# noc-lab/sac-expert

Measured on AMD Instinct MI355X. Metric: SAC gradient-steps/sec (batch=256, 256x2 MLP), higher is better.
Workload: dtype f32; 1 GPU; HalfCheetah-v3-shaped synthetic buffer, SAC twin-Q + actor + alpha update (no model), fp32; obs_dim=17, act_dim=6, batch=256, buffer_rows=1000000, parallelism=replicas x1 (independent seeds, no collective), seeds_per_gpu=1, sampler=NumPy-legacy MT19937 stream on device (bit-exact indices)

## Files before the change

sac-expert_amd/csrc/k_sac.hip:

```cpp
#include <hip/hip_runtime.h>
#include <cstddef>
#include <cstdio>
#include <cstdlib>
#include <type_traits>
#include <utility>
#include <math.h>
#include "sacx_internal.h"

#pragma clang fp contract(off)

namespace sacx {

typedef float floatx4 __attribute__((ext_vector_type(4)));


typedef __bf16 bf16x8_t __attribute__((ext_vector_type(8)));
__device__ __forceinline__ floatx4 mfma_bf16_2slab(const float (&a0)[4], const float (&a1)[4], const float (&b0)[4],
                                                   const float (&b1)[4], floatx4 c) {
    const bf16x8_t av = {(__bf16)a0[0], (__bf16)a0[1], (__bf16)a0[2], (__bf16)a0[3],
                         (__bf16)a1[0], (__bf16)a1[1], (__bf16)a1[2], (__bf16)a1[3]};
    const bf16x8_t bv = {(__bf16)b0[0], (__bf16)b0[1], (__bf16)b0[2], (__bf16)b0[3],
                         (__bf16)b1[0], (__bf16)b1[1], (__bf16)b1[2], (__bf16)b1[3]};
    return __builtin_amdgcn_mfma_f32_16x16x32_bf16(av, bv, c, 0, 0, 0);
}
// ... 651 lines not shown
            if (f.nt > 0) ak = 0.5f * ak;
            const float lk = ak / (float)f.mb;
            tot = k == 0 ? lk : tot + lk;
        }
        const int64_t seq = f.ctl->mfit_seq;
        f.mstats[(size_t)(seq % f.mstats_cap) * 2] = tot;
        f.mstats[(size_t)(seq % f.mstats_cap) * 2 + 1] = (float)seq;
        f.ctl->t_model = t_model + 1;
        f.ctl->mfit_seq = seq + 1;
    }
}

template <int MODE, int NQ>
__device__ __forceinline__ void qhead_block(const QHeadArgs& q, int block, int64_t so, const FinalArgs* fin = nullptr);
template <int NQ, int OW = 0, int FIN = 0>
__device__ __forceinline__ void actor_head_body(const HeadArgs& h, const FinalArgs& f, int block, int64_t so,
                                                const FinalArgs& ffin);
template <int NQ, int OW = 0>
__device__ __forceinline__ void actor_head_body(const HeadArgs& h, const FinalArgs& f, int block, int64_t so) {
    actor_head_body<NQ, OW, 0>(h, f, block, so, f);
}

__device__ __forceinline__ int xcd_tile(int b, int T) {
    const int x = b & 7, j = b >> 3, q = T >> 3, r = T & 7;
    return x * q + (x < r ? x : r) + j;
}

struct HeadPre {
    float xs[4], u, ls, am, ad, bias;
    float4 pv[4];
};
__device__ __forceinline__ void head_pre_load(const HeadArgs& hd, const GemmProb& g, int m0, int64_t so, bool parts,
                                              HeadPre& p) {
    const int t = threadIdx.x, row = t >> 4, col = t & 15;
    const int A = hd.A, Aout = hd.Aout, H1 = hd.H1, S = g.K - A;
    HeadSeg sg = hd.seg[0];
    reloc(sg, so);
    const bool rok = m0 + row < g.M;
    const __amdgpu_buffer_rsrc_t rx = make_rsrc(g.A, 0x7fffffffu);
#pragma unroll
    for (int q = 0; q < 4; ++q) p.xs[q] = bload(rx, boff(rok && col + 16 * q < S, (m0 + row) * g.lda + col + 16 * q));
    const bool jok = col < A;
    p.u = bload(rs(sg.noise), boff(jok && rok, (m0 + row - sg.r0) * A + col));
    p.ls = bload(rs(sr(hd.logstd, so)), boff(jok && !hd.per_state_std, col));
    p.am = bload(rs(sr(hd.a_mean, so)), boff(jok, col));
    p.ad = bload(rs(sr(hd.a_den, so)), boff(jok, col));
    const __amdgpu_buffer_rsrc_t rw3 = make_rsrc(sr(hd.W3, so), 0x7fffffffu);
    p.bias = bload(rw3, boff(col < Aout, H1 * Aout + col));
    if (parts) {
        const __amdgpu_buffer_rsrc_t rp = rs(sr(hd.part, so));
        const bool pok = rok && col < Aout;
#pragma unroll
        for (int i = 0; i < 4; ++i) p.pv[i] = bload4(rp, boff(pok && 4 * i < hd.tq, ((m0 + row) * Aout + col) * hd.tq + 4 * i));
    }
}
__device__ __forceinline__ float head_pre_mu(const HeadPre& p) {
    float v = 0.f;
#pragma unroll
    for (int i = 0; i < 4; ++i) {
        v = v + p.pv[i].x; v = v + p.pv[i].y; v = v + p.pv[i].z; v = v + p.pv[i].w;
    }
    return v + p.bias;
}
__device__ __forceinline__ void head_pre_finish(const HeadArgs& hd, const GemmProb& g, int m0, int tn,
                                                float (&As)[16][68], const HeadPre& p, float mu, int64_t so) {
    const int t = threadIdx.x, lane = t & 63;
    const int row = t >> 4, col = t & 15;
    const int A = hd.A, S = g.K - A;
    HeadSeg sg = hd.seg[0];
    reloc(sg, so);
    const bool rok = m0 + row < g.M;
    const bool jok = col < A;
    const float lv = __shfl(mu, (lane & ~15) | min(col + A, 15), 64);
    const float lraw = hd.per_state_std ? lv : p.ls;
    float nv = 0.f, nc = 0.f, pin = 0.f;
    if (jok) {
        const float l = fminf(fmaxf(lraw, -5.f), 2.f);
        const float sd = expf(l);
        const float x = mu + sd * p.u;
        const float th = tanhf(x);
        const float pi = hd.lim * th;
        const float z = (x - mu) / expf(l);
        nv = z * z + 2.f * l + LOG2PI_F;
        nc = 2.f * ((LN2_F - x) - softplus_f(-2.f * x));
        pin = (pi - p.am) / p.ad;
    }
    nv += __shfl_xor(nv, 8, 16);
    nv += __shfl_xor(nv, 4, 16);
    nv += __shfl_xor(nv, 2, 16);
    nv += __shfl_xor(nv, 1, 16);
    nc += __shfl_xor(nc, 8, 16);
    nc += __shfl_xor(nc, 4, 16);
    nc += __shfl_xor(nc, 2, 16);
    nc += __shfl_xor(nc, 1, 16);
    if (tn == 0 && col == 0 && rok && sg.nlp_out != nullptr) sg.nlp_out[m0 + row - sg.r0] = 0.5f * nv + nc;
#pragma unroll
    for (int q = 0; q < 4; ++q)
        if (col + 16 * q < S) As[row][col + 16 * q] = p.xs[q];
    if (jok) As[row][S + col] = pin;
}

template <bool SYNC = true>
__device__ __forceinline__ void head_prologue(const HeadArgs& hd, const GemmProb& g, int m0, int tn,
                                              float (&As)[16][68], float (&red)[4][4][64], int64_t so) {
    const int t = threadIdx.x, wave = t >> 6, lane = t & 63, r = lane & 15, grp = lane >> 4;
    const int row = t >> 4, col = t & 15;
    const int Aout = hd.Aout, H1 = hd.H1;
    HeadPre p;
    head_pre_load(hd, g, m0, so, hd.part != nullptr, p);
    float mu;
    if (hd.part != nullptr) {
        mu = head_pre_mu(p);
    } else {
        const __amdgpu_buffer_rsrc_t rw3 = make_rsrc(sr(hd.W3, so), 0x7fffffffu);
        const __amdgpu_buffer_rsrc_t rh = make_rsrc(sr(hd.H2, so), 0x7fffffffu);
        const int nIt = H1 >> 4, per = (nIt + 3) >> 2, i0 = wave * per, i1 = min(nIt, i0 + per);
        const bool hm = m0 + r < g.M, wn = r < Aout;
        floatx4 c0 = {0.f, 0.f, 0.f, 0.f}, c1 = {0.f, 0.f, 0.f, 0.f};
        for (int it = i0; it < i1; it += 4) {
            float a[4][4], b[4][4];
#pragma unroll
            for (int u4 = 0; u4 < 4; ++u4) {
                const bool ok = it + u4 < i1;
                const int k0 = (it + u4) * 16 + grp * 4;
                const float4 v = bload4(rh, boff(ok && hm, (m0 + r) * hd.ldh + k0));
                a[u4][0] = v.x; a[u4][1] = v.y; a[u4][2] = v.z; a[u4][3] = v.w;
#pragma unroll
                for (int j = 0; j < 4; ++j) b[u4][j] = bload(rw3, boff(ok && wn, (k0 + j) * Aout + r));
            }
            __builtin_amdgcn_sched_barrier(0);
#pragma unroll
            for (int u4 = 0; u4 < 4; ++u4) {
                c0 = __builtin_amdgcn_mfma_f32_16x16x4f32(a[u4][0], b[u4][0], c0, 0, 0, 0);
                c1 = __builtin_amdgcn_mfma_f32_16x16x4f32(a[u4][1], b[u4][1], c1, 0, 0, 0);
                c0 = __builtin_amdgcn_mfma_f32_16x16x4f32(a[u4][2], b[u4][2], c0, 0, 0, 0);
                c1 = __builtin_amdgcn_mfma_f32_16x16x4f32(a[u4][3], b[u4][3], c1, 0, 0, 0);
            }
        }
        const floatx4 acc = c0 + c1;
#pragma unroll
        for (int q = 0; q < 4; ++q) red[wave][q][lane] = acc[q];
        __syncthreads();
        const int L = ((row >> 2) << 4) | col, R = row & 3;
        float v = red[0][R][L] + red[1][R][L];
        v = v + red[2][R][L];
        v = v + red[3][R][L];
        mu = v + p.bias;
    }
    head_pre_finish(hd, g, m0, tn, As, p, mu, so);
    if constexpr (SYNC) __syncthreads();
}

__device__ __forceinline__ void head_bwd_prologue(HeadBwdArgs hb, int m0, int tn, float (&d3s)[16][17], int64_t so) {
    reloc(hb, so);
    const int t = threadIdx.x, lane = t & 63, row = t >> 4, col = t & 15;
    const int B = hb.B, A = hb.A;
    const int m = m0 + row;
    const bool rok = m < B + hb.ne, jok = col < A, ok = rok && jok;
    const bool pol = m < B;
    const int ci = m * A + col;
    const float ct = bload(rs(hb.c_t), boff(ok, ci));
    const float sd = bload(rs(hb.c_std), boff(ok, ci));
    const float u = bload(rs(hb.c_u), boff(ok, ci));
    const float mk = bload(rs(hb.c_mask), boff(ok, ci));
    const float ad = bload(rs(pol ? hb.a_den : hb.ma_den), boff(jok, col));
    const __amdgpu_buffer_rsrc_t rg = rs(hb.gpol);
    const float g0 = bload(rg, boff(rok && pol, m));
    const float g1 = bload(rg, boff(rok && pol, B + m));
    const float alpha = bload(rs(hb.alpha), 0u);
    const float eps = hb.ctl != nullptr ? bload(rs(reinterpret_cast<const float*>(hb.ctl)),
                                               (uint32_t)offsetof(Ctl, epsilon)) : 0.f;
    const __amdgpu_buffer_rsrc_t rp = rs(hb.part), rm = rs(hb.mpart);
    const int tq = hb.tq, tqm = hb.tqm, e = m - B;
    float4 v0[4], v1[4], vm[8];
#pragma unroll
    for (int i = 0; i < 4; ++i) {
        const bool iok = ok && pol && 4 * i < tq;
        v0[i] = bload4(rp, boff(iok, (m * A + col) * tq + 4 * i));
        v1[i] = bload4(rp, boff(iok, ((B + m) * A + col) * tq + 4 * i));
    }
#pragma unroll
    for (int i = 0; i < 8; ++i) vm[i] = bload4(rm, boff(ok && !pol && 4 * i < tqm, (e * A + col) * tqm + 4 * i));
// ... 401 lines not shown
    static_assert(GEMM_MAXP == 8, "one pin per problem's tile_begin");
    const uint32_t kf = khdr_flags(kh);
    if (kf & 0x80u) {
        total_tiles = (int)khdr_field(kh, 0);
        row_blocks = (int)khdr_field(kh, 1);
        tb[0] = 0;
#pragma unroll
        for (int i = 1; i < GEMM_MAXP; ++i) tb[i] = (int)khdr_field(kh, i + 1);
        nprob = (int)(kf & 15u);
        has_final = (int)((kf >> 4) & 3u);
        xcd_map = (int)((kf >> 6) & 1u);
    } else {
        has_final = ga.has_final; row_blocks = ga.row_blocks; total_tiles = ga.total_tiles;
        xcd_map = ga.xcd_map; nprob = ga.nprob;
#pragma unroll
        for (int i = 0; i < GEMM_MAXP; ++i) tb[i] = ga.probs[i].tile_begin;
        asm volatile("" ::"s"(has_final), "s"(row_blocks), "s"(total_tiles), "s"(xcd_map), "s"(nprob),
                     "s"(tb[1]), "s"(tb[2]), "s"(tb[3]), "s"(tb[4]), "s"(tb[5]), "s"(tb[6]), "s"(tb[7]));
    }
    int tile = (int)blockIdx.x - (has_final ? 1 : 0);
    if (tile < 0) {
        FinalArgs f = ga.fin;
        reloc(f, so);
        finalize_update(f, f.nred);
        return;
    }
    if constexpr (gemm_rows_head(MODE, ROWK)) {
        if (tile < row_blocks) {
            actor_head_body<NQ>(ga.head, ga.hfin, ga.head_block0 + tile, so);
            return;
        }
        tile -= row_blocks;
    }
    if (tile >= total_tiles) {
        if constexpr (gemm_rows_qhead(MODE, ROWK)) {
            qhead_block<gemm_qhead_mode(ROWK), NQ>(ga.qh, tile - total_tiles, so, ROWK == GR_QHEAD ? &ga.fin : nullptr);
        } else if constexpr (gemm_rows_mfinal(ROWK)) {
            if (ga.has_mfinal == 2) {
                FinalArgs f = ga.fin;
                reloc(f, so);
                bc_finalize(f);
            } else if (ga.has_mfinal) {
                mfit_final(ga.mfin, &ga.adam, ga.p_stride);
            }
        }
        return;
    }
    if (xcd_map) tile = xcd_tile(tile, total_tiles);
    int p = 0;
#pragma unroll
    for (int i = 1; i < GEMM_MAXP; ++i)
        if (i < nprob && tile >= tb[i]) p = i;
    GemmProb g = ga.probs[p];
    if constexpr (MODE == GM_FWD && ROWK == GR_ACTOR_HEAD) {
        const HeadArgs& hd = ga.head;
        const HeadSeg& s0 = hd.seg[0];
        asm volatile("" ::"s"(g.A), "s"(g.B), "s"(g.lda), "s"(g.ldb), "s"(g.M), "s"(g.N), "s"(g.K), "s"(g.tiles_n),
                     "s"(g.tile_begin), "s"(g.act), "s"(g.bias), "s"(g.headp), "s"(hd.H2), "s"(hd.W3), "s"(hd.logstd),
                     "s"(hd.a_mean), "s"(hd.a_den), "s"(hd.ldh), "s"(hd.H1), "s"(hd.A), "s"(hd.Aout),
                     "s"(hd.per_state_std), "s"(hd.lim), "s"(s0.r0), "s"(s0.noise), "s"(s0.nlp_out), "s"(g.vec),
                     "s"(hd.part), "s"(hd.tq));
    } else if constexpr (MODE == GM_FWD && ROWK == GR_HEAD_PART) {
        asm volatile("" ::"s"(g.A), "s"(g.B), "s"(g.lda), "s"(g.ldb), "s"(g.M), "s"(g.N), "s"(g.K), "s"(g.tiles_n),
                     "s"(g.tile_begin), "s"(g.act), "s"(g.bias), "s"(g.vec), "s"(g.C), "s"(g.ldc),
                     "s"(g.pw), "s"(g.ppart), "s"(g.pw_ld), "s"(g.pw_cs), "s"(g.pw_n));
    } else if constexpr (MODE == GM_FWD) {
        asm volatile("" ::"s"(g.A), "s"(g.B), "s"(g.lda), "s"(g.ldb), "s"(g.M), "s"(g.N), "s"(g.K), "s"(g.tiles_n),
                     "s"(g.tile_begin), "s"(g.act), "s"(g.bias), "s"(g.mse), "s"(g.se_raw), "s"(g.spe_raw),
                     "s"(g.dmean), "s"(g.dden), "s"(g.headp), "s"(g.vec));
    } else if constexpr (MODE == GM_DX && ROWK == GR_PIQHEAD) {
// ... 55 lines not shown
        e2 = g.P[pidx + 2 * ga.p_stride];
        e3 = bload(make_rsrc(g.T, g.T != nullptr ? 0x7fffffffu : 0u), (uint32_t)pidx * 4u);
    }
    EpiScalars es{};
    if constexpr (MODE == GM_DW || (MODE == GM_FWD && ROWK == GR_MSE_HEAD))
        es = epi_scalars(sr(ga.ctl, so), g.group);
    constexpr bool PART = gemm_rows_part(MODE, ROWK);
    float pwv[8];
    if constexpr (PART) {
        const __amdgpu_buffer_rsrc_t rpw = rs(g.pw);
#pragma unroll
        for (int j = 0; j < 8; ++j) pwv[j] = bload(rpw, boff(j < g.pw_n && nn < g.N, j * g.pw_ld + nnc * g.pw_cs));
    }

    const int nIt = (g.K + 15) >> 4;
    const int per = (nIt + 3) >> 2;
    const int it0 = wave * per;
    const int it1 = min(nIt, it0 + per);
    const int m = m0 + r, n = n0 + r;
    const bool mok = m < g.M, nok = n < g.N;

    const __amdgpu_buffer_rsrc_t ra = make_rsrc(g.A, 0x7fffffffu);
    const __amdgpu_buffer_rsrc_t rb = make_rsrc(g.B, 0x7fffffffu);
    const __amdgpu_buffer_rsrc_t rw = rs(g.wgen);
    floatx4 acc0 = {0.f, 0.f, 0.f, 0.f};
    floatx4 acc1 = {0.f, 0.f, 0.f, 0.f};
    __shared__ float As[16][68];
    bool a_lds = false;
    if constexpr (MODE == GM_FWD && ROWK == GR_ACTOR_HEAD) {
        if (g.headp) {
            float bp[4];
            const int k0 = it0 * 16 + grp * 4;
            load_b<BKC, false, false>(rb, g, n, nok, it0 < it1 ? k0 : (1 << 30), bp);
            head_prologue(ga.head, g, m0, tn, As, red, so);
            if (it0 < it1) {
                float a[4];
#pragma unroll
                for (int j = 0; j < 4; ++j) a[j] = (k0 + j < g.K) ? As[r][k0 + j] : 0.f;
                if constexpr (BF) {
                    const float z[4] = {0.f, 0.f, 0.f, 0.f};
                    acc0 = mfma_bf16_2slab(a, z, bp, z, acc0);
                } else {
                    acc0 = __builtin_amdgcn_mfma_f32_16x16x4f32(a[0], bp[0], acc0, 0, 0, 0);
                    acc1 = __builtin_amdgcn_mfma_f32_16x16x4f32(a[1], bp[1], acc1, 0, 0, 0);
                    acc0 = __builtin_amdgcn_mfma_f32_16x16x4f32(a[2], bp[2], acc0, 0, 0, 0);
                    acc1 = __builtin_amdgcn_mfma_f32_16x16x4f32(a[3], bp[3], acc1, 0, 0, 0);
                }
            }
            a_lds = true;
        }
    }
    __shared__ float d3s[ROWK == GR_HEAD_BWD ? 16 : 1][17];
    if constexpr (MODE == GM_DX && ROWK == GR_HEAD_BWD) {
        auto hbw_loop = [&](auto vt) {
            constexpr bool V = decltype(vt)::value;
            const int Aout = ga.hbw.Aout;
            float a[4][4], b[4][4], w[4][2];
#pragma unroll
            for (int u = 0; u < 4; ++u) {
                const int it = it0 + u;
                const int k0 = it * 16 + grp * 4;
                const int k0e = it < it1 ? k0 : (1 << 30);
                load_a<true, V, false>(ra, g, m, mok, k0e, a[u], rw);
                load_b<true, V>(rb, g, n, nok, k0e, b[u]);
                const int kr = it * 16 + r;
#pragma unroll
                for (int s = 0; s < 2; ++s)
// ... 753 lines not shown

template <bool PK, bool T32>
static void launch_gemm_t(const GemmArgs& a, hipStream_t s) {
    const std::make_integer_sequence<int, GR_COUNT> rows;
    switch (a.mode) {
    case GM_FWD: return launch_gemm_rows<GM_FWD, PK, T32>(a, s, rows);
    case GM_DX: return launch_gemm_rows<GM_DX, PK, T32>(a, s, rows);
    case GM_DW: return launch_gemm_rows<GM_DW, PK, T32>(a, s, rows);
    default: gemm_variant_die(a);
    }
}

#ifndef SACX_FWD2_NW
#define SACX_FWD2_NW 16
#endif

#ifndef SACX_DW_DIAG_XBF
#define SACX_DW_DIAG_XBF 0
#endif
#ifndef SACX_FWD2_STAMP
#define SACX_FWD2_STAMP 0
#endif

#define F2_STAMP(P)                                                                          \
    do {                                                                                     \
        if (SACX_FWD2_STAMP == (P) && ga.ktime != nullptr) {                                 \
            __syncthreads();                                                                 \
            if (threadIdx.x == 0) {                                                          \
                ga.ktime[2 * f2_slot(ga, g1, lt, HEAD)] = t0;                                \
                ga.ktime[2 * f2_slot(ga, g1, lt, HEAD) + 1] = __builtin_amdgcn_s_memrealtime(); \
            }                                                                                \
        }                                                                                    \
    } while (0)
__device__ __forceinline__ int f2_slot(const GemmArgs& ga, const GemmProb& g1, int lt, bool head) {
    return (head ? ga.row_blocks : 0) + g1.tile_begin + lt;
}
template <int VEC, int NW, bool HEAD, int FIN = 0, int H0X = 256, bool GATHER = false>
__global__ __launch_bounds__(NW * 64, HEAD ? 2 * NW / 4 : 1) void k_fwd2(GemmArgs ga) {
    constexpr int L0T = (H0X / 16) / NW, CTW = 16 / NW, PU = H0X / 64;
    const uint64_t t0 = __builtin_amdgcn_s_memrealtime();
    __shared__ float hs[16][H0X + 4];
    __shared__ float red2[4][4][4][64];
    int p = (int)blockIdx.y;
    if constexpr (HEAD) {
        if (p == 0) {
            const int tile = (int)blockIdx.x;
            if (tile >= ga.row_blocks) return;
            const int blk = ga.head_block0 + (NW / 4) * tile;
            actor_head_body<4, 0, FIN>(ga.head, ga.hfin, blk, 0, ga.fin);
            if (ga.ktime != nullptr) {
                __syncthreads();
                if (threadIdx.x == 0) {
                    ga.ktime[2 * tile] = t0;
                    ga.ktime[2 * tile + 1] = __builtin_amdgcn_s_memrealtime();
                }
            }
            return;
        }
        --p;
    }
    const GemmProb g0 = ga.probs[2 * p], g1 = ga.probs[2 * p + 1];
    const int lt = (int)blockIdx.x;
    if (lt >= ((g1.M + 15) >> 4) * g1.tiles_n) return;
    if (SACX_FWD2_STAMP == 3) {
        asm volatile("" ::"s"(g0.N), "s"(g1.N), "s"(g0.A), "s"(g1.B));
        F2_STAMP(3);
    }
    const int tm = lt / g1.tiles_n, cg = lt - tm * g1.tiles_n;
    const int m0 = tm * 16;
    const int wave = wave_id(), lane = threadIdx.x & 63, r = lane & 15, grp = lane >> 4;
    const int kq = wave & 3, ch = wave >> 2;
    const bool headp = HEAD && g0.headp;
    const int m = m0 + r;
    const bool mok = m < g0.M;
    const int H0 = g0.N, N1 = g1.N;
    const int nIt0 = (g0.K + 15) >> 4;
    const int per1 = (H0 + 63) >> 6;

    HeadPre hpre;
    if constexpr (HEAD)
        if (headp && threadIdx.x < 256) head_pre_load(ga.head, g0, m0, 0, true, hpre);
    const __amdgpu_buffer_rsrc_t rx = make_rsrc(g0.A, 0x7fffffffu);
    const __amdgpu_buffer_rsrc_t rw0 = make_rsrc(g0.B, 0x7fffffffu);
    const __amdgpu_buffer_rsrc_t rw1 = make_rsrc(g1.B, 0x7fffffffu);
    const __amdgpu_buffer_rsrc_t rnull = rs(nullptr);
    float xa[2][4];
    const float* trec = nullptr;
    if constexpr (GATHER) {
        const MGatherArgs& mg = ga.mg;
        const int64_t seq = mg.ctl->mfit_seq, start = mg.ctl->start;
        const int32_t* ir = mg.idx_ring + (seq % mg.idx_cap) * (int64_t)(mg.nm * mg.mb) + (int64_t)p * mg.mb;
        auto rec_of = [&](int rr) {
            int64_t phys = start + ir[min(rr, g0.M - 1)];
            phys = phys >= mg.cap ? phys - mg.cap : phys;
            return mg.replay + phys * (int64_t)mg.stride;
        };
        const float* grow = rec_of(m);
        trec = rec_of(m0 + ((threadIdx.x & 255) >> 4));
#pragma unroll
        for (int s2 = 0; s2 < 2; ++s2) {
            const int k0 = s2 < nIt0 ? s2 * 16 + grp * 4 : (1 << 30);
            const bool live = mok && k0 < g0.K;
            const int kb = k0 < g0.K ? k0 : 0;
            float raw[4];
            if constexpr (VEC == 1) {
                const float4 q = *reinterpret_cast<const float4*>(grow + kb);
                raw[0] = q.x; raw[1] = q.y; raw[2] = q.z; raw[3] = q.w;
            } else {
#pragma unroll
                for (int j = 0; j < 4; ++j) raw[j] = grow[min(kb + j, g0.K - 1)];
            }
#pragma unroll
            for (int j = 0; j < 4; ++j) {
                const int kc = min(kb + j, g0.K - 1);
                const float* mu = kc < mg.S ? mg.s_mean + kc : mg.a_mean + (kc - mg.S);
                const float* den = kc < mg.S ? mg.s_den + kc : mg.a_den + (kc - mg.S);
                float x = (raw[j] - *mu) / *den;
                asm("" : "+v"(x));
                xa[s2][j] = (live && kb + j < g0.K) ? x : 0.f;
            }
            if (cg == 0 && wave == 0 && mok && k0 < g0.lda)
                *reinterpret_cast<float4*>(const_cast<float*>(g0.A) + (size_t)m * g0.lda + k0) =
                    float4{xa[s2][0], xa[s2][1], xa[s2][2], xa[s2][3]};
        }
    } else {
#pragma unroll
        for (int s2 = 0; s2 < 2; ++s2)
            load_a<true, VEC == 1, false>(rx, g0, m, mok && !headp, s2 < nIt0 ? s2 * 16 + grp * 4 : (1 << 30), xa[s2], rnull);
    }
    float w0[L0T][2][4], b0[L0T];
#pragma unroll
    for (int i = 0; i < L0T; ++i) {
        const int c = wave + NW * i;
        const int nc = 16 * c + r;
        const bool cok = nc < H0;
#pragma unroll
        for (int s2 = 0; s2 < 2; ++s2) load_b<false, false>(rw0, g0, nc, cok, s2 < nIt0 && cok ? s2 * 16 + grp * 4 : (1 << 30), w0[i][s2]);
        b0[i] = bload(rs(g0.bias), boff(cok, nc));
    }
    float w1[CTW][PU][4];
#pragma unroll
    for (int j2 = 0; j2 < CTW; ++j2) {
        const int ct = CTW * ch + j2;
        const int n1 = 64 * cg + 16 * ct + r;
        const bool nok = n1 < N1;
#pragma unroll
        for (int u = 0; u < PU; ++u) {
            const int it = kq * per1 + u;
            load_b<false, false>(rw1, g1, n1, nok, u < per1 ? it * 16 + grp * 4 : (1 << 30), w1[j2][u]);
        }
    }
    const int te = threadIdx.x & 255, eh = threadIdx.x >> 8;
    const int row = te >> 4, col = te & 15;
    float b1[CTW];
    constexpr int NPW = HEAD ? 1 : 8;
    float pwv[CTW][NPW];
#pragma unroll
    for (int j2 = 0; j2 < CTW; ++j2) {
        const int nn = 64 * cg + 16 * (CTW * eh + j2) + col;
        b1[j2] = bload(rs(g1.bias), boff(nn < N1, nn));
        if constexpr (!HEAD) {
            const __amdgpu_buffer_rsrc_t rpw = rs(ga.rowk == GR_HEAD_PART ? g1.pw : nullptr);
#pragma unroll
            for (int j = 0; j < NPW; ++j)
                pwv[j2][j] = bload(rpw, boff(j < g1.pw_n && nn < N1, j * g1.pw_ld + min(nn, N1 - 1) * g1.pw_cs));
        }
    }
    __builtin_amdgcn_sched_barrier(0);
    if constexpr (GATHER) {
        const MGatherArgs& mg = ga.mg;
        const int S = mg.S, A = mg.A, tcol = 16 * eh + col, mmr = m0 + row;
        if (cg == 0 && mmr < g0.M && tcol <= S) {
            const int c = tcol;
            const float traw0 = c < S ? trec[S + A + c] : trec[2 * S + A];
            const float traw1 = c < S ? trec[c] : 0.f;
            const float tmu = c < S ? mg.d_mean[c] : mg.r_norm[0];
            const float tden = c < S ? mg.d_den[c] : mg.r_norm[1];
            float y = c < S ? ((traw0 - traw1) - tmu) / tden : (traw0 - tmu) / tden;
            const float cl = c < S ? mg.clip_d : mg.clip_r;
            if (cl > 0.f) y = fminf(fmaxf(y, -cl), cl);
            mg.T[(size_t)(p * mg.mb + mmr) * (S + 1) + c] = y;
        }
    }
    if constexpr (HEAD) {
        __shared__ float As[16][68];
        if (headp) {
            if (SACX_FWD2_STAMP == 6) {
                const float mu6 = head_pre_mu(hpre);
                asm volatile("" ::"v"(mu6), "v"(hpre.xs[3]), "v"(hpre.u));
                F2_STAMP(6);
            }
            if (threadIdx.x < 256) head_pre_finish(ga.head, g0, m0, cg, As, hpre, head_pre_mu(hpre), 0);
            __syncthreads();
            F2_STAMP(5);
#pragma unroll
            for (int s2 = 0; s2 < 2; ++s2)
#pragma unroll
                for (int j = 0; j < 4; ++j) {
                    const int k = s2 * 16 + grp * 4 + j;
                    xa[s2][j] = (s2 < nIt0 && k < g0.K) ? As[r][k] : 0.f;
                }
        }
    }

#pragma unroll
    for (int i = 0; i < L0T; ++i) {
        const int c = wave + NW * i;
        if (16 * c >= H0) break;
        floatx4 ps[2];
#pragma unroll
        for (int s2 = 0; s2 < 2; ++s2) {
            floatx4 x0 = {0.f, 0.f, 0.f, 0.f}, x1 = {0.f, 0.f, 0.f, 0.f};
            x0 = __builtin_amdgcn_mfma_f32_16x16x4f32(xa[s2][0], w0[i][s2][0], x0, 0, 0, 0);
            x1 = __builtin_amdgcn_mfma_f32_16x16x4f32(xa[s2][1], w0[i][s2][1], x1, 0, 0, 0);
            x0 = __builtin_amdgcn_mfma_f32_16x16x4f32(xa[s2][2], w0[i][s2][2], x0, 0, 0, 0);
            x1 = __builtin_amdgcn_mfma_f32_16x16x4f32(xa[s2][3], w0[i][s2][3], x1, 0, 0, 0);
            ps[s2] = x0 + x1;
        }
        const floatx4 v4 = ((ps[0] + ps[1]) + floatx4{0.f, 0.f, 0.f, 0.f}) + floatx4{0.f, 0.f, 0.f, 0.f};
        const int nc = 16 * c + r;
#pragma unroll
        for (int q = 0; q < 4; ++q) {
            const float h = act_f(v4[q] + b0[i], g0.act);
            hs[4 * grp + q][nc] = h;
            const int mm = m0 + 4 * grp + q;
            if (cg == 0 && mm < g0.M && nc < H0) st_out(&g0.C[(size_t)mm * g0.ldc + nc], h);
        }
    }
    F2_STAMP(1);
    __syncthreads();

    float a1[PU][4];
#pragma unroll
    for (int u = 0; u < PU; ++u) {
        const int k0 = (kq * per1 + u) * 16 + grp * 4;
        const float4 q4 = u < per1 ? *reinterpret_cast<const float4*>(&hs[r][k0]) : float4{0.f, 0.f, 0.f, 0.f};
        a1[u][0] = q4.x; a1[u][1] = q4.y; a1[u][2] = q4.z; a1[u][3] = q4.w;
    }
#pragma unroll
    for (int j2 = 0; j2 < CTW; ++j2) {
        floatx4 acc0 = {0.f, 0.f, 0.f, 0.f}, acc1 = {0.f, 0.f, 0.f, 0.f};
#pragma unroll
        for (int u = 0; u < PU; ++u) {
            if (u >= per1) break;
            acc0 = __builtin_amdgcn_mfma_f32_16x16x4f32(a1[u][0], w1[j2][u][0], acc0, 0, 0, 0);
            acc1 = __builtin_amdgcn_mfma_f32_16x16x4f32(a1[u][1], w1[j2][u][1], acc1, 0, 0, 0);
            acc0 = __builtin_amdgcn_mfma_f32_16x16x4f32(a1[u][2], w1[j2][u][2], acc0, 0, 0, 0);
            acc1 = __builtin_amdgcn_mfma_f32_16x16x4f32(a1[u][3], w1[j2][u][3], acc1, 0, 0, 0);
        }
        const floatx4 acc = acc0 + acc1;
#pragma unroll
// ... 1719 lines not shown
    hipLaunchKernelGGL(k_softmax_pick, dim3((p.m + 3) / 4), dim3(256), 0, s, p);
}

template <bool PF>
__global__ __launch_bounds__(1024) void k_softmax_rows(ActRowArgs g) {
    __shared__ ActShared L;
    const int row = blockIdx.x;
    act_rows_body<PF, false>(g, row, L);
    if (threadIdx.x < 64) {
        const int lane = threadIdx.x;
        const float l = lane < g.A ? L.outs[lane] : 0.f;
        const int idx = softmax_pick(l, g.noise ? g.noise + (size_t)row * g.A : nullptr, lane, g.A);
        if (lane == 0) reinterpret_cast<int32_t*>(g.out)[row] = idx;
    }
    act_rows_done(g.done);
}

void launch_softmax_rows(const ActRowArgs& a, int m, hipStream_t s) {
    const bool pf = a.S <= 128 && a.H0 <= 256 && a.H1 <= 256 && a.Aout <= 16;
    if (pf) hipLaunchKernelGGL(k_softmax_rows<true>, dim3(m), dim3(1024), 0, s, a);
    else hipLaunchKernelGGL(k_softmax_rows<false>, dim3(m), dim3(1024), 0, s, a);
}

template <int MODE, int NQ>
__device__ __forceinline__ void qhead_block(const QHeadArgs& q_in, int block, int64_t so, const FinalArgs* fin) {
    __shared__ float buf[4][512];
    QHeadArgs q = q_in;
    reloc(q, so);
    const int wave = wave_id(), lane = threadIdx.x & 63;
    const int row = block * 4 + wave;
    const int B = q.B, H1 = q.H1;
    if (row < B) {
        constexpr int nnet = (MODE == 0) ? 4 : 2;
        float alpha;
        if (MODE == 0 && fin != nullptr && fin->pre != nullptr) {
            const FinalArgs& f = *fin;
            const AfinPre* P = f.pre;
            const float* const xs[1] = {f.red};
            const int ns[1] = {f.nred};
            float p0[1];
            strided_sums<1>(xs, ns, p0);
            const float a_old = P->a_old, a_m = P->a_m, a_v = P->a_v;
            const int64_t t_sac = P->t_sac, seq = P->seq0, nts = P->nts, tsi = P->tsi;
            const float m_ent = wave_sum(p0[0]) / (float)f.B;
            const int64_t tnew = t_sac + 1;
            const float g = -m_ent;
            const float lr_t = adam_lr(f.adam, GRP_ALPHA, tnew);
            const float b1 = 0.9f, b2 = 0.999f, eps = 1e-7f;
            const float mm = a_m + (g - a_m) * (1.f - b1);
            const float vv = a_v + (g * g - a_v) * (1.f - b2);
            float an = a_old - (mm * lr_t) / (sqrtf(vv) + eps);
            an = fmaxf(an, 1e-5f);
            alpha = an;
            if (block == 0 && wave == 0 && lane == 0) {
                *f.alpha_m = mm;
                *f.alpha_v = vv;
                *f.alpha = an;
                float* st = f.stats + (size_t)(seq % f.stats_cap) * 8;
                st[3] = -a_old * m_ent;
                st[4] = an;
                st[6] = -(m_ent - f.target_entropy);
                st[7] = (float)seq;
                Ctl* ctl = f.ctl;
                ctl->t_sac = tnew;
                ctl->num_timesteps = nts + tsi;
                ctl->step_seq = seq + 1;
            }
        } else {
            alpha = *q.alpha;
        }
        const float nlp_r = q.nlp[row];
        float r_r = 0.f, d_r = 0.f, rd = 1.f;
        if (MODE == 0) {
            r_r = q.r[row];
            d_r = q.d[row];
            rd = *q.ret_den;
        }
        float hv[4][NQ];
        float wv[4][NQ];
        float bias[4];
        const __amdgpu_buffer_rsrc_t rH = rs(q.H2);
#pragma unroll
        for (int k = 0; k < nnet; ++k) {
            load_row(rH, (k * B + row) * H1, H1, hv[k]);
            const __amdgpu_buffer_rsrc_t rW = rs(q.W3[k]);
            load_row(rW, 0, H1, wv[k]);
            bias[k] = bload(rW, (uint32_t)H1 * 4u);
        }
        float out[4];
#pragma unroll
        for (int k = 0; k < nnet; ++k) {
            float p = 0.f;
#pragma unroll
            for (int i = 0; i < NQ; ++i) p = fmaf(hv[k][i], wv[k][i], p);
            out[k] = wave_sum(p) + bias[k];
        }
        float g0, g1;
        if constexpr (MODE == 0) {
            const float v0 = out[0] * rd, v1 = out[1] * rd;
            const float nv = fminf(v0, v1) + alpha * nlp_r;
            const float y = r_r + q.gamma * ((1.f - d_r) * nv);
            const float e0 = out[2] - y, e1 = out[3] - y;
            const float invB = 1.f / (float)B;
            g0 = e0 * invB;
            g1 = e1 * invB;
            if (lane == 0) {
                q.loss_rows[row] = 0.5f * (e0 * e0);
                q.loss_rows[B + row] = 0.5f * (e1 * e1);
                q.g[row] = g0;
                q.g[B + row] = g1;
            }
        } else {
            const float q0 = out[0], q1 = out[1];
            const float minq = fminf(q0, q1);
            if (lane == 0) q.loss_rows[row] = (-alpha) * nlp_r - minq;
            const float gmin = -q.w_sac * (1.f / (float)B);
            const float s0 = q0 < q1 ? 1.f : (q0 == q1 ? 0.5f : 0.f);
            const float s1 = q1 < q0 ? 1.f : (q0 == q1 ? 0.5f : 0.f);
            g0 = gmin * s0;
            g1 = gmin * s1;
            if (lane == 0 && q.g != nullptr) {
// ... 1608 lines not shown
```

sac-expert_amd/csrc/sacx.cpp:

```cpp
#include "sacx.h"
#include "sacx_internal.h"
#include "vcritic.h"
#include "trpo.h"
#include "mt_jump.h"
#include "sampler_sched.h"

#include <rccl/rccl.h>

#include <algorithm>
#include <cmath>
#include <cstdio>
#include <cstdlib>
#include <cstddef>
#include <chrono>
#include <cstring>
#include <map>
#include <stdexcept>
#include <string>
#include <tuple>
#include <vector>

using namespace sacx;

namespace {
// ... 1587 lines not shown
    };
    actor_fwd(actor_pass_ws(h, Xa, h->Ra, 0, h->Ra), "actor.fwd", "actor.ln");
    const char* fh = std::getenv("SACX_FUSE_HEAD");
    const bool fuse_head = Aout <= 16 && S + A <= 64 && H1 % 16 == 0 && H1 <= 512 &&
                           (fh ? std::atoi(fh) != 0 : h->plan_seeds < 4);
    const char* fhb = std::getenv("SACX_FOLD_HBW");
    const int tq = (Hc0 + 15) / 16;
    const bool fold_hbw = fold_hbw_shape(h) && (fhb ? std::atoi(fhb) != 0 : h->tile32_plan == 0);
    HeadArgs head_fused{};
    if (fuse_head) {
        HeadArgs& a = head_fused;
        a = head_args(h, Ha2, hpart(0), true);
        a.nseg = 1;
        a.seg[0] = {0, B, 0, 0, noise_t, nullptr, W("ws.nlp_t")};
        a.total_rows = h->Ra;
        a.cache_row0 = 1 << 30;
        a.cache_row1 = 1 << 30;
        if (eo) {
            a.nseg = 2;
            a.seg[1] = {2 * B, 2 * B + h->ne, 1, 0, noise_e, Xm, nullptr};
            a.cache_row0 = B;
            a.cache_row1 = h->Ra;
        }
    } else {
        plan.push_back(actor_head_launch(h, slot, hpart(0)));
    }
    {
        std::vector<GemmProb> p0, p1;
        for (int k = 0; k < 4; ++k) {
            p0.push_back(critic_fwd_prob(h, qn[k], k < 2 ? Xt : Xq, "ws.Hq", k, 0));
            p1.push_back(critic_fwd_prob(h, qn[k], nullptr, "ws.Hq", k, 1));
        }
        if (fuse_head) {
            p0[0].headp = p0[1].headp = 1;
            add_gemm(h, plan, "q.fwd0+actor.head", p0);
            Launch& L = plan.back();
            set_rows(L, GR_ACTOR_HEAD);
            L.gemm.head = head_fused;
            L.gemm.head_block0 = eo ? (2 * B) / 4 : ((h->Ra + 3) & ~3) / 4;
            L.gemm.row_blocks = eo ? (h->Ra + 3) / 4 - (2 * B) / 4 : 0;
            L.grid += L.gemm.row_blocks;
            L.flops += 2.0 * B * H1 * Aout;
            L.bytes += 4.0 * B * (H1 + 6.0 * A);
            L.frees_slot = true;
            for (int k = 0; eo && k < nm; ++k) p1.push_back(model_fwd_prob(h, Xm, k, 0));
            add_gemm(h, plan, "q.fwd1", p1);
            if (h->fwd2 && !eo) fuse_fwd2(h, plan, "q.fwd01+actor.head");
        } else {
            for (int k = 0; eo && k < nm; ++k) {
                p0.push_back(model_fwd_prob(h, Xm, k, 0));
                p1.push_back(model_fwd_prob(h, Xm, k, 1));
            }
            fwd_pair("q.fwd", p0, p1);
        }
    }
    {
        std::vector<GemmProb> pb;
        for (int k = 0; k < 2; ++k) {
            GemmProb p = critic_dx_prob(h, qk(k), "ws.Hq", 2 + k, "ws.Dq", k, 1, true);
            p.wgen = W(qk(k) + ".l2");
            p.gen_act = c1;
            pb.push_back(p);
        }
        add_gemm(h, plan, "q.head+critic.bwd1", pb);
        Launch& L = plan.back();
        set_rows(L, GR_QHEAD);
        L.gemm.row_blocks = (B + 3) / 4;
// ... 773 lines not shown
    std::vector<std::pair<int, int>> rowspan;
    std::vector<std::vector<int>> cls;
    bool rows = false;
};

std::vector<std::pair<int, int>> sampler_batches(const sacx_handle* h, int G) {
    if (h->grow > h->nbatch && G >= kSamplerGrowMinG) return sampler_batches_grown(G, h->grow);
    return sampler_batches_fixed(G, h->nbatch);
}

int chain_body(sacx_handle* h, int G, bool with_rng, int skip_kind, KTimeMap* kt) {
    auto emit = [&](const Launch& L, hipStream_t st) {
        const bool timed = kt && (L.kind == Launch::GEMM || (kt->rows && (L.kind == Launch::AHEAD || L.kind == Launch::ABWD)));
        if (timed) {
            Launch C = L;
            const int fin_wg = C.gemm.has_final && C.gemm.mode != GM_FWD2 ? 1 : 0;
            const int nwg1 = L.kind == Launch::GEMM
                                 ? (C.gemm.mode != GM_FWD2 && !C.gemm.has_mfinal
                                        ? gemm_workgroups(C.gemm)
                                        : C.gemm.total_tiles + fin_wg + (C.gemm.rowk ? C.gemm.row_blocks : 0))
                                 : (L.kind == Launch::AHEAD ? (C.head.total_rows + 3) / 4 : C.grid);
            const int nwg = nwg1 * h->seeds;
            if (kt->used + 2 * nwg <= kt->cap) {
                uint64_t* p = kt->base + kt->used;
                if (L.kind == Launch::GEMM) C.gemm.ktime = p;
                else if (L.kind == Launch::AHEAD) C.head.ktime = p;
                else C.ab.ktime = p;
                kt->spans.push_back({kt->used, nwg});
                kt->names.push_back(C.name);
                kt->is_gemm.push_back(L.kind == Launch::GEMM);
                if (L.kind != Launch::GEMM) kt->rowspan.push_back({0, 0});
                else if (C.gemm.rowk == GR_ACTOR_HEAD)
                    kt->rowspan.push_back({fin_wg, fin_wg + C.gemm.row_blocks});
                else kt->rowspan.push_back({C.gemm.total_tiles + fin_wg, nwg1});
                std::vector<int> cb;
                if (L.kind == Launch::GEMM && C.gemm.mode == GM_FWD2) {
                    const int nn = C.gemm.nprob / 2, r0 = C.gemm.rowk == GR_PAIR_HEAD ? C.gemm.row_blocks : 0;
                    for (int i = 0; i < nn; ++i) cb.push_back(r0 + C.gemm.probs[nn + i].tile_begin);
                }
                kt->cls.push_back(cb);
                kt->used += 2 * nwg;
            }
            enqueue(C, h, st);
        } else {
            enqueue(L, h, st);
        }
    };
    hipStream_t cs = h->cap_stream, rs = h->rng_stream;
    hipEvent_t* evR = h->events.data();
    hipEvent_t* evS = h->events.data() + G;
    hipEvent_t* evF = h->events.data() + 2 * G;
    hipEvent_t evFork = h->events[3 * G];
    if (with_rng) {
        const bool merge = h->dp_ranks == 0;
        HIPCHK(h, hipEventRecord(evFork, cs));
        HIPCHK(h, hipStreamWaitEvent(rs, evFork, 0));
        const std::vector<std::pair<int, int>> batches = sampler_batches(h, G);
        const int nslot = h->nslot;
        for (int b = 0; b < (int)batches.size(); ++b) {
            const int s0 = batches[b].first, n = batches[b].second - s0;
            if ((b + 1 < (int)batches.size() && batches[b + 1].first != batches[b].second) || n < 1 ||
                s0 % nslot + n > nslot || (s0 > 0 && sampler_emit_after(batches[b], nslot) >= s0))
                return fail(h, "internal: sampler batches");
        }
        auto prologue = [&](int b) {
            const int j0 = batches[b].first, n = batches[b].second - j0;
// ... 3207 lines not shown
```

Baseline: 17530 gradient-steps/s.

## Overlap actor-head prologue with layer-0 MFMA and reorder qhead row blocks

```diff
diff --git a/sac-expert_amd/csrc/k_sac.hip b/sac-expert_amd/csrc/k_sac.hip
--- a/sac-expert_amd/csrc/k_sac.hip
+++ b/sac-expert_amd/csrc/k_sac.hip
@@ -707,7 +707,7 @@
 };
 __device__ __forceinline__ void head_pre_load(const HeadArgs& hd, const GemmProb& g, int m0, int64_t so, bool parts,
                                               HeadPre& p) {
-    const int t = threadIdx.x, row = t >> 4, col = t & 15;
+    const int t = threadIdx.x & 255, row = t >> 4, col = t & 15;
     const int A = hd.A, Aout = hd.Aout, H1 = hd.H1, S = g.K - A;
     HeadSeg sg = hd.seg[0];
     reloc(sg, so);
@@ -737,9 +737,10 @@
     }
     return v + p.bias;
 }
-__device__ __forceinline__ void head_pre_finish(const HeadArgs& hd, const GemmProb& g, int m0, int tn,
+template <int PART = 3>
+__device__ __forceinline__ void head_pre_finish(const HeadArgs& hd, const GemmProb& g, int m0, bool nlp,
                                                 float (&As)[16][68], const HeadPre& p, float mu, int64_t so) {
-    const int t = threadIdx.x, lane = t & 63;
+    const int t = threadIdx.x & 255, lane = t & 63;
     const int row = t >> 4, col = t & 15;
     const int A = hd.A, S = g.K - A;
     HeadSeg sg = hd.seg[0];
@@ -753,30 +754,38 @@
         const float l = fminf(fmaxf(lraw, -5.f), 2.f);
         const float sd = expf(l);
         const float x = mu + sd * p.u;
-        const float th = tanhf(x);
-        const float pi = hd.lim * th;
-        const float z = (x - mu) / expf(l);
-        nv = z * z + 2.f * l + LOG2PI_F;
-        nc = 2.f * ((LN2_F - x) - softplus_f(-2.f * x));
-        pin = (pi - p.am) / p.ad;
-    }
-    nv += __shfl_xor(nv, 8, 16);
-    nv += __shfl_xor(nv, 4, 16);
-    nv += __shfl_xor(nv, 2, 16);
-    nv += __shfl_xor(nv, 1, 16);
-    nc += __shfl_xor(nc, 8, 16);
-    nc += __shfl_xor(nc, 4, 16);
-    nc += __shfl_xor(nc, 2, 16);
-    nc += __shfl_xor(nc, 1, 16);
-    if (tn == 0 && col == 0 && rok && sg.nlp_out != nullptr) sg.nlp_out[m0 + row - sg.r0] = 0.5f * nv + nc;
-#pragma unroll
-    for (int q = 0; q < 4; ++q)
-        if (col + 16 * q < S) As[row][col + 16 * q] = p.xs[q];
-    if (jok) As[row][S + col] = pin;
+        if ((PART & 2) && nlp) {
+            const float z = (x - mu) / expf(l);
+            nv = z * z + 2.f * l + LOG2PI_F;
+            nc = 2.f * ((LN2_F - x) - softplus_f(-2.f * x));
+        }
+        if (PART & 1) {
+            const float th = tanhf(x);
+            const float pi = hd.lim * th;
+            pin = (pi - p.am) / p.ad;
+        }
+    }
+    if ((PART & 2) && nlp) {
+        nv += __shfl_xor(nv, 8, 16);
+        nv += __shfl_xor(nv, 4, 16);
+        nv += __shfl_xor(nv, 2, 16);
+        nv += __shfl_xor(nv, 1, 16);
+        nc += __shfl_xor(nc, 8, 16);
+        nc += __shfl_xor(nc, 4, 16);
+        nc += __shfl_xor(nc, 2, 16);
+        nc += __shfl_xor(nc, 1, 16);
+        if (col == 0 && rok && sg.nlp_out != nullptr) sg.nlp_out[m0 + row - sg.r0] = 0.5f * nv + nc;
+    }
+    if (PART & 1) {
+#pragma unroll
+        for (int q = 0; q < 4; ++q)
+            if (col + 16 * q < S) As[row][col + 16 * q] = p.xs[q];
+        if (jok) As[row][S + col] = pin;
+    }
 }
 
 template <bool SYNC = true>
-__device__ __forceinline__ void head_prologue(const HeadArgs& hd, const GemmProb& g, int m0, int tn,
+__device__ __forceinline__ void head_prologue(const HeadArgs& hd, const GemmProb& g, int m0, bool nlp,
                                               float (&As)[16][68], float (&red)[4][4][64], int64_t so) {
     const int t = threadIdx.x, wave = t >> 6, lane = t & 63, r = lane & 15, grp = lane >> 4;
     const int row = t >> 4, col = t & 15;
@@ -822,7 +831,7 @@
         v = v + red[3][R][L];
         mu = v + p.bias;
     }
-    head_pre_finish(hd, g, m0, tn, As, p, mu, so);
+    head_pre_finish(hd, g, m0, nlp, As, p, mu, so);
     if constexpr (SYNC) __syncthreads();
 }
 
@@ -1290,10 +1299,15 @@
         }
         tile -= row_blocks;
     }
+    if constexpr (gemm_rows_qhead(MODE, ROWK)) {
+        if (tile < row_blocks) {
+            qhead_block<gemm_qhead_mode(ROWK), NQ>(ga.qh, tile, so, ROWK == GR_QHEAD ? &ga.fin : nullptr);
+            return;
+        }
+        tile -= row_blocks;
+    }
     if (tile >= total_tiles) {
-        if constexpr (gemm_rows_qhead(MODE, ROWK)) {
-            qhead_block<gemm_qhead_mode(ROWK), NQ>(ga.qh, tile - total_tiles, so, ROWK == GR_QHEAD ? &ga.fin : nullptr);
-        } else if constexpr (gemm_rows_mfinal(ROWK)) {
+        if constexpr (gemm_rows_mfinal(ROWK)) {
             if (ga.has_mfinal == 2) {
                 FinalArgs f = ga.fin;
                 reloc(f, so);
@@ -1415,7 +1429,7 @@
             float bp[4];
             const int k0 = it0 * 16 + grp * 4;
             load_b<BKC, false, false>(rb, g, n, nok, it0 < it1 ? k0 : (1 << 30), bp);
-            head_prologue(ga.head, g, m0, tn, As, red, so);
+            head_prologue(ga.head, g, m0, tn == 0 && g.headp == 1, As, red, so);
             if (it0 < it1) {
                 float a[4];
 #pragma unroll
@@ -2235,6 +2249,14 @@
             }                                                                                \
         }                                                                                    \
     } while (0)
+__device__ __forceinline__ floatx4 fwd2_l0_slab(const float (&a)[4], const float (&w)[4]) {
+    floatx4 x0 = {0.f, 0.f, 0.f, 0.f}, x1 = {0.f, 0.f, 0.f, 0.f};
+    x0 = __builtin_amdgcn_mfma_f32_16x16x4f32(a[0], w[0], x0, 0, 0, 0);
+    x1 = __builtin_amdgcn_mfma_f32_16x16x4f32(a[1], w[1], x1, 0, 0, 0);
+    x0 = __builtin_amdgcn_mfma_f32_16x16x4f32(a[2], w[2], x0, 0, 0, 0);
+    x1 = __builtin_amdgcn_mfma_f32_16x16x4f32(a[3], w[3], x1, 0, 0, 0);
+    return x0 + x1;
+}
 __device__ __forceinline__ int f2_slot(const GemmArgs& ga, const GemmProb& g1, int lt, bool head) {
     return (head ? ga.row_blocks : 0) + g1.tile_begin + lt;
 }
@@ -2280,9 +2302,11 @@
     const int nIt0 = (g0.K + 15) >> 4;
     const int per1 = (H0 + 63) >> 6;
 
+    const bool nlps = headp && cg == 0 && g0.headp == 1;
+    const bool l0e = headp && g0.K - ga.head.A >= 16;
     HeadPre hpre;
     if constexpr (HEAD)
-        if (headp && threadIdx.x < 256) head_pre_load(ga.head, g0, m0, 0, true, hpre);
+        if (headp && (threadIdx.x < 256 || nlps)) head_pre_load(ga.head, g0, m0, 0, true, hpre);
     const __amdgpu_buffer_rsrc_t rx = make_rsrc(g0.A, 0x7fffffffu);
     const __amdgpu_buffer_rsrc_t rw0 = make_rsrc(g0.B, 0x7fffffffu);
     const __amdgpu_buffer_rsrc_t rw1 = make_rsrc(g1.B, 0x7fffffffu);
@@ -2329,7 +2353,7 @@
     } else {
 #pragma unroll
         for (int s2 = 0; s2 < 2; ++s2)
-            load_a<true, VEC == 1, false>(rx, g0, m, mok && !headp, s2 < nIt0 ? s2 * 16 + grp * 4 : (1 << 30), xa[s2], rnull);
+            load_a<true, VEC == 1, false>(rx, g0, m, mok && (!headp || (s2 == 0 && l0e)), s2 < nIt0 ? s2 * 16 + grp * 4 : (1 << 30), xa[s2], rnull);
     }
     float w0[L0T][2][4], b0[L0T];
 #pragma unroll
@@ -2370,6 +2394,7 @@
         }
     }
     __builtin_amdgcn_sched_barrier(0);
+    floatx4 ps0[HEAD ? L0T : 1];
     if constexpr (GATHER) {
         const MGatherArgs& mg = ga.mg;
         const int S = mg.S, A = mg.A, tcol = 16 * eh + col, mmr = m0 + row;
@@ -2388,21 +2413,29 @@
     if constexpr (HEAD) {
         __shared__ float As[16][68];
         if (headp) {
+            if (l0e) {
+#pragma unroll
+                for (int i = 0; i < L0T; ++i)
+                    if (16 * (wave + NW * i) < H0) ps0[i] = fwd2_l0_slab(xa[0], w0[i][0]);
+            }
             if (SACX_FWD2_STAMP == 6) {
                 const float mu6 = head_pre_mu(hpre);
                 asm volatile("" ::"v"(mu6), "v"(hpre.xs[3]), "v"(hpre.u));
                 F2_STAMP(6);
             }
-            if (threadIdx.x < 256) head_pre_finish(ga.head, g0, m0, cg, As, hpre, head_pre_mu(hpre), 0);
+            if (threadIdx.x < 256) head_pre_finish<1>(ga.head, g0, m0, false, As, hpre, head_pre_mu(hpre), 0);
+            else if (nlps) head_pre_finish<2>(ga.head, g0, m0, true, As, hpre, head_pre_mu(hpre), 0);
             __syncthreads();
             F2_STAMP(5);
 #pragma unroll
-            for (int s2 = 0; s2 < 2; ++s2)
+            for (int s2 = 0; s2 < 2; ++s2) {
+                if (s2 == 0 && l0e) continue;
 #pragma unroll
                 for (int j = 0; j < 4; ++j) {
                     const int k = s2 * 16 + grp * 4 + j;
                     xa[s2][j] = (s2 < nIt0 && k < g0.K) ? As[r][k] : 0.f;
                 }
+            }
         }
     }
 
@@ -2411,15 +2444,9 @@
         const int c = wave + NW * i;
         if (16 * c >= H0) break;
         floatx4 ps[2];
-#pragma unroll
-        for (int s2 = 0; s2 < 2; ++s2) {
-            floatx4 x0 = {0.f, 0.f, 0.f, 0.f}, x1 = {0.f, 0.f, 0.f, 0.f};
-            x0 = __builtin_amdgcn_mfma_f32_16x16x4f32(xa[s2][0], w0[i][s2][0], x0, 0, 0, 0);
-            x1 = __builtin_amdgcn_mfma_f32_16x16x4f32(xa[s2][1], w0[i][s2][1], x1, 0, 0, 0);
-            x0 = __builtin_amdgcn_mfma_f32_16x16x4f32(xa[s2][2], w0[i][s2][2], x0, 0, 0, 0);
-            x1 = __builtin_amdgcn_mfma_f32_16x16x4f32(xa[s2][3], w0[i][s2][3], x1, 0, 0, 0);
-            ps[s2] = x0 + x1;
-        }
+        if (HEAD && l0e) ps[0] = ps0[i];
+        else ps[0] = fwd2_l0_slab(xa[0], w0[i][0]);
+        ps[1] = fwd2_l0_slab(xa[1], w0[i][1]);
         const floatx4 v4 = ((ps[0] + ps[1]) + floatx4{0.f, 0.f, 0.f, 0.f}) + floatx4{0.f, 0.f, 0.f, 0.f};
         const int nc = 16 * c + r;
 #pragma unroll
@@ -4205,6 +4232,30 @@
     const int B = q.B, H1 = q.H1;
     if (row < B) {
         constexpr int nnet = (MODE == 0) ? 4 : 2;
+        float nlp_r, r_r = 0.f, d_r = 0.f, rd = 1.f;
+        float hv[4][NQ];
+        float wv[4][NQ];
+        float bias[4];
+        auto request_rows = [&]() {
+            nlp_r = q.nlp[row];
+            if (MODE == 0) {
+                r_r = q.r[row];
+                d_r = q.d[row];
+                rd = *q.ret_den;
+            }
+            const __amdgpu_buffer_rsrc_t rH = rs(q.H2);
+#pragma unroll
+            for (int k = 0; k < nnet; ++k) {
+                load_row(rH, (k * B + row) * H1, H1, hv[k]);
+                const __amdgpu_buffer_rsrc_t rW = rs(q.W3[k]);
+                load_row(rW, 0, H1, wv[k]);
+                bias[k] = bload(rW, (uint32_t)H1 * 4u);
+            }
+        };
+        if constexpr (NQ <= 4) {
+            request_rows();
+            __builtin_amdgcn_sched_barrier(0);
+        }
         float alpha;
         if (MODE == 0 && fin != nullptr && fin->pre != nullptr) {
             const FinalArgs& f = *fin;
@@ -4242,24 +4293,7 @@
         } else {
             alpha = *q.alpha;
         }
-        const float nlp_r = q.nlp[row];
-        float r_r = 0.f, d_r = 0.f, rd = 1.f;
-        if (MODE == 0) {
-            r_r = q.r[row];
-            d_r = q.d[row];
-            rd = *q.ret_den;
-        }
-        float hv[4][NQ];
-        float wv[4][NQ];
-        float bias[4];
-        const __amdgpu_buffer_rsrc_t rH = rs(q.H2);
-#pragma unroll
-        for (int k = 0; k < nnet; ++k) {
-            load_row(rH, (k * B + row) * H1, H1, hv[k]);
-            const __amdgpu_buffer_rsrc_t rW = rs(q.W3[k]);
-            load_row(rW, 0, H1, wv[k]);
-            bias[k] = bload(rW, (uint32_t)H1 * 4u);
-        }
+        if constexpr (NQ > 4) request_rows();
         float out[4];
 #pragma unroll
         for (int k = 0; k < nnet; ++k) {
diff --git a/sac-expert_amd/csrc/sacx.cpp b/sac-expert_amd/csrc/sacx.cpp
--- a/sac-expert_amd/csrc/sacx.cpp
+++ b/sac-expert_amd/csrc/sacx.cpp
@@ -1643,7 +1643,8 @@
             p1.push_back(critic_fwd_prob(h, qn[k], nullptr, "ws.Hq", k, 1));
         }
         if (fuse_head) {
-            p0[0].headp = p0[1].headp = 1;
+            p0[0].headp = 1;
+            p0[1].headp = 2;
             add_gemm(h, plan, "q.fwd0+actor.head", p0);
             Launch& L = plan.back();
             set_rows(L, GR_ACTOR_HEAD);
@@ -2483,6 +2484,8 @@
                 if (L.kind != Launch::GEMM) kt->rowspan.push_back({0, 0});
                 else if (C.gemm.rowk == GR_ACTOR_HEAD)
                     kt->rowspan.push_back({fin_wg, fin_wg + C.gemm.row_blocks});
+                else if (gemm_rows_qhead(C.gemm.mode, C.gemm.rowk))
+                    kt->rowspan.push_back({0, C.gemm.row_blocks});
                 else kt->rowspan.push_back({C.gemm.total_tiles + fin_wg, nwg1});
                 std::vector<int> cb;
                 if (L.kind == Launch::GEMM && C.gemm.mode == GM_FWD2) {
```

Result: no change. 17600 gradient-steps/s, median of 6 (+0.4%).
